# LoganWilliams1/mhm2_kmer_analysis_v2

Measured on AMD Instinct MI355X. Metric: k-mers/sec (kcount stage) at k=21, higher is better.
Workload: dtype u64

## Files before the change

### mhm2_kmer_analysis_v2_amd/csrc/kc_bucketed.hpp

```cpp
#pragma once
#include "kc_kernels.hpp"

namespace kc {

constexpr int WGB = 1024;
constexpr int SUPER_SPAN = 16 * WGB - PRE - POST;
using TileSuper = TileGeo<WGB, SUPER_SPAN>;
static_assert(TileSuper::GPT == 1 && TileSuper::NGROUP == WGB, "one group per thread");
constexpr int PMAX = 1024;
constexpr int GMAX = 512;

template <int NL> struct Rnd {
  static constexpr int RPOS = NL == 1 ? 16 : NL == 2 ? 8 : 4;
  static constexpr int RPOS_READS = NL == 1 ? 8 : NL <= 3 ? 4 : 2;
  static constexpr size_t STAGE = ((size_t)WGB * RPOS + 64) * NL * 8;
  static constexpr size_t STAGE_READS = ((size_t)WGB * RPOS_READS + 64) * NL * 8;
};

struct Geom {
  uint32_t G, P1, P2, S;
  uint32_t log2CH1, log2CH2;
  uint32_t L1MAX, L2MAX;
  uint32_t A1;
  uint32_t A2;
// ... 409 lines not shown
    Lh ^= kc_feistel_f(Rh, 0, K);
    Rh ^= kc_feistel_f(Lh, 1, K);
    Lh ^= kc_feistel_f(Rh, 2, K);
    const uint64_t mix = ((uint64_t)Lh << K) | Rh;
    lo[j] = (uint32_t)mix;
    bk[j] = valid ? ((uint32_t)(mix >> (2 * K - gm.la)) | (le << 10) | (re << 13)) : ~0u;
  }
}

template <int K, int RPOS, class TL>
__device__ __forceinline__ uint32_t cut_run_fixed(const TL &L, int lp0, bool active, uint64_t (&rec)[RPOS], uint64_t (&h)[RPOS]) {
  constexpr int NB = RPOS + K + 1;
  static_assert(NB <= 32 && RPOS % 8 == 0 && PRE % 8 == 0, "the window must fit one word and never start word-aligned");
  const uint64_t *W = reinterpret_cast<const uint64_t *>(L.codes);
  const uint32_t *OK = reinterpret_cast<const uint32_t *>(L.ok);
  const int p = lp0 - 1, q = p >> 5, s = p & 31;
  const uint64_t w0 = W[q], w1 = W[q + 1];
  const uint32_t ok0 = OK[q], ok1 = OK[q + 1], g0 = L.gap[q], g1 = L.gap[q + 1];
  const uint64_t Wn = (w0 << (2 * s)) | (w1 >> (64 - 2 * s));
  const uint32_t nok = ~__builtin_amdgcn_alignbit(ok1, ok0, (uint32_t)s);
  const uint32_t gapw = __builtin_amdgcn_alignbit(g1, g0, (uint32_t)s);
  const uint64_t Rn = kc_rc_word(Wn) << (64 - 2 * NB);
  constexpr uint64_t MID = ((1ULL << (2 * K)) - 1ULL) << 2;
  constexpr uint64_t CMP = (K & 1) ? (MID | 3ULL) : MID;
  uint32_t okm = 0;
#pragma unroll
  for (int j = 0; j < RPOS; j++) {
    const uint64_t x = Wn >> (64 - 2 * (j + K + 2)), y = Rn >> (64 - 2 * (RPOS - 1 - j + K + 2));
    const bool swap = (y & CMP) < (x & CMP);
    const uint64_t sel = swap ? y : x;
    const uint32_t na = (nok >> j) & 1u, nb = (nok >> (j + K + 1)) & 1u;
    const uint32_t le = ((uint32_t)(sel >> (2 * K + 2)) & 3u) | ((swap ? nb : na) << 2);
    const uint32_t re = ((uint32_t)sel & 3u) | ((swap ? na : nb) << 2);
    const uint64_t key = (sel >> 2) << (64 - 2 * K);
    const uint64_t kk[1] = {key};
    h[j] = kc_hash<1>(kk);
    rec[j] = key | (uint64_t)((le & 4u) ? 4u : le) | ((uint64_t)((re & 4u) ? 4u : re) << 3);
    const bool valid = active && ((gapw >> (j + 1)) & ((1u << (K + 1)) - 1u)) == 0u;
    okm |= valid ? (1u << j) : 0u;
  }
  return okm;
}

template <int NL, int FMT, bool CP, bool SH>
__global__ __launch_bounds__(WGB) void kc_l1_reads_kernel(ExtractArgs a, Geom gm, BucketBufs bb, uint64_t nsuper, uint32_t rot,
                                                          uint64_t *ctrs, uint64_t *cb) {
  extern __shared__ __align__(16) uint8_t smem[];
  L1LDS &L = *reinterpret_cast<L1LDS *>(smem);
  uint64_t *sorted = reinterpret_cast<uint64_t *>(smem + ((sizeof(L1LDS) + 15) & ~size_t(15)));
  uint16_t *sbucket = CP ? nullptr : reinterpret_cast<uint16_t *>(smem + ((sizeof(L1LDS) + 15) & ~size_t(15)) + Rnd<NL>::STAGE_READS);
  constexpr int RPOS = Rnd<NL>::RPOS_READS;
  const int tid = threadIdx.x;
  const uint32_t g = (blockIdx.x + rot) % gm.G, P1 = gm.P1;
  ChainDest D = l1_dest<NL>(gm, bb, g);
#ifdef KC_STAMPS
  unsigned long long tprev_ = __builtin_amdgcn_s_memtime();
  D.stamps = cb + 8;
  D.tprev = &tprev_;
#endif
  ChainState cst = split_load_state(L.sp, P1, bb.cnt1 + (size_t)g * P1, D.chain, D.LMAX, D.log2CH, bb.used1[g], bb.used1[gm.G + g]);
  __syncthreads();
  uint32_t n_ins = 0;
  int buf = 0;
  TileRaw<TileSuper> raw;
  auto first_of = [&](uint64_t st) -> uint64_t { return (FMT != FMT_SEQBLOCK && st < nsuper) ? a.tile_first[st] : 0; };
  tile_prefetch<FMT, TileSuper>(raw, a, a.pos0 + (int64_t)blockIdx.x * SUPER_SPAN, tid, first_of(blockIdx.x), blockIdx.x < nsuper);
  uint64_t next_first = first_of((uint64_t)blockIdx.x + gridDim.x);
  constexpr int RUNS = SUPER_SPAN / RPOS;
  static_assert(SUPER_SPAN % RPOS == 0, "runs must tile the span");
  constexpr int NROUND = (RUNS + WGB - 1) / WGB;
  for (int64_t it = -1;; it++) {
    const uint64_t st = (uint64_t)blockIdx.x + (uint64_t)(it < 0 ? 0 : it) * gridDim.x;
    const bool work = it >= 0;
    if (work && st >= nsuper) break;
#pragma unroll 1
    for (int round = 0; round < NROUND; round++) {
      uint64_t rec[RPOS][NL];
      uint32_t br[RPOS];
      uint32_t total = 0;
      if (work) {
      const int run_id = round * WGB + tid;
      const bool active = run_id < RUNS;
      const int lp0 = PRE + (active ? run_id : 0) * RPOS;
      KmerRun<NL> run;
      run_begin<NL>(run, L.tile, lp0, a.k);
#pragma unroll
      for (int j = 0; j < RPOS; j++) {
        uint64_t h = 0;
        uint32_t owner = 0;
        bool valid = run_kmer<NL, !CP>(run, j, lp0, a.k, rec[j], h, SH ? a.rank_n : 1u, SH ? a.reference_owner : 0u, SH ? &owner : nullptr) && active;
        if (SH) {
          if (CP && !a.reference_owner) {
            uint64_t key[NL];
#pragma unroll
            for (int w = 0; w < NL; w++) key[w] = rec[j][w];
            key[NL - 1] &= ~KC_EXT_MASK;
            owner = kc_owner_of_hash(kc_hash<NL>(key), a.rank_n);
          }
          valid = valid && owner == a.rank_me;
        }
        if (CP) rec[j][0] = cp_mix_rec(rec[j][0], gm);
        br[j] = valid ? (CP ? cp_b1(rec[j][0], gm) : hash_b1(h, gm)) : ~0u;
        if (j + 1 < RPOS) run_advance<NL>(run, j, lp0, a.k);
      }
#pragma unroll
      for (int j = 0; j < RPOS; j++) {
        const bool valid = br[j] != ~0u;
        const uint32_t rank = hist_rank(L.sp, buf, br[j] & (PMAX - 1), valid);
        br[j] = valid ? (br[j] | (rank << 10)) : ~0u;
        n_ins += valid ? 1u : 0u;
      }
      KC_SPLIT_STAMP(0)
      lds_barrier();
      total = split_stage<NL, RPOS>(
          L.sp, sorted, sbucket, buf, P1,
          [&](int j, uint64_t (&o)[NL]) {
#pragma unroll
            for (int w = 0; w < NL; w++) o[w] = rec[j][w];
          },
          br, D, cst);
      }
      if (round == NROUND - 1) {
        const uint64_t nst = work ? st + gridDim.x : st;
        tile_encode<FMT, TileSuper>(L.tile, raw, a, a.pos0 + (int64_t)nst * SUPER_SPAN, ctrs, tid, nst < nsuper);
        tile_prefetch<FMT, TileSuper>(raw, a, a.pos0 + (int64_t)(nst + gridDim.x) * SUPER_SPAN, tid, next_first, nst + gridDim.x < nsuper);
        next_first = first_of(nst + 2 * (uint64_t)gridDim.x);
        KC_SPLIT_STAMP(5)
      }
      if (work) {
        split_copy_out<NL>(
            L.sp, sorted, sbucket, total, D, [&](const uint64_t (&r)[NL]) { return cp_b1(r[0], gm); },
            [&](uint32_t, const uint64_t (&r)[NL]) { l1_overflow<NL, CP>(gm, bb, cb, r); },
            [&](size_t i, const uint64_t (&r)[NL]) { store_words<NL>(D.arena, i, r); });
        buf ^= 1;
      }
    }
  }
  if ((uint32_t)tid < P1) bb.cnt1[(size_t)g * P1 + tid] = cst.cur;
  if (tid == 0) {
    bb.used1[g] = min(L.sp.arena_used, gm.A1);
    bb.used1[gm.G + g] = min(L.sp.arena_top, gm.A1);
  }
  for (int o = 32; o > 0; o >>= 1) n_ins += __shfl_down(n_ins, o);
  if (lane_id() == 0 && n_ins) atomicAdd((unsigned long long *)&ctrs[CTR_INSERTED], (unsigned long long)n_ins);
}

constexpr int R16 = 16;
constexpr uint32_t ST16_MAIN = (uint32_t)WGB * R16 + PMAX;
constexpr uint32_t ST16_SLOTS = ST16_MAIN + 64;
static_assert(SUPER_SPAN % R16 == 0 && SUPER_SPAN / R16 <= WGB, "one run of sixteen positions per thread covers the super-tile");
static_assert(ST16_MAIN < 65536, "staging positions fit 16 bits");
constexpr size_t l1x16_lds_bytes() { return ((sizeof(L1LDS) + 15) & ~size_t(15)) + (size_t)ST16_SLOTS * 6; }

template <class MidFn>
__device__ __forceinline__ uint32_t split_stage_pairs(SplitLDS &L, uint32_t *slo, uint16_t *sbk, int buf, uint32_t P, const uint32_t (&lo)[R16],
                                                      const uint32_t (&br)[R16], const ChainDest &D, ChainState &st, MidFn mid) {
  const int tid = fresh_tid();
  KC_SPLIT_STAMP(1)
  const uint32_t v = ((uint32_t)tid < P) ? L.hist[buf][tid] : 0u;
  const uint32_t excl = block_excl_scan((v + 1u) & ~1u, L.scan);
  const uint32_t CHm = (1u << D.log2CH) - 1u;
  if ((uint32_t)tid < P) {
    const uint32_t base = st.cur;
    uint32_t fit = v;
    const uint64_t room = ((uint64_t)D.LMAX << D.log2CH) - base;
    if ((uint64_t)fit > room) fit = (uint32_t)room;
    const uint32_t have = (base + CHm) >> D.log2CH;
    uint32_t k = ((base + fit + CHm) >> D.log2CH) - have, a = 0;
    if (k) {
      const bool own = (uint32_t)tid >= D.own_lo && (uint32_t)tid < D.own_hi;
      if (own) {
        a = atomicAdd(&L.arena_used, k);
        const uint32_t left = D.arena_cap - min(D.arena_cap, L.arena_top);
        if (a + k > left) {
          k = a < left ? left - a : 0;
          const uint64_t cap = ((uint64_t)(have + k) << D.log2CH) - base;
          if ((uint64_t)fit > cap) fit = (uint32_t)cap;
        }
      } else {
        const uint32_t t = atomicAdd(&L.arena_top, k);
        const uint32_t left = D.arena_cap - min(D.arena_cap, L.arena_used);
        if (t + k > left) {
          k = 0;
          const uint64_t cap = ((uint64_t)have << D.log2CH) - base;
          if ((uint64_t)fit > cap) fit = (uint32_t)cap;
        } else {
          a = D.arena_cap - t - k;
        }
      }
      uint32_t *ch = D.chain + (size_t)tid * D.LMAX + have;
      for (uint32_t i = 0; i < k; i++) ch[i] = D.arena_base + a + i;
    }
    uint4 d;
    d.x = ((st.last - D.arena_base - (base >> D.log2CH)) << D.log2CH) + base - excl;
    d.y = ((a - have) << D.log2CH) + base - excl;
    d.z = excl | (v << 16);
    d.w = fit | (((base & CHm) ? min(fit, (CHm + 1u) - (base & CHm)) : 0u) << 16);
    L.dst[tid] = d;
    if (k) st.last = D.arena_base + a + k - 1;
    st.cur = base + fit;
    L.hist[buf][tid] = excl;
    L.hist[buf ^ 1][tid] = 0;
  }
  lds_barrier();
  KC_SPLIT_STAMP(2)
  const uint32_t total = L.scan.total;
#pragma unroll
  for (int j0 = 0; j0 < R16; j0 += 8) {
    uint32_t pos[8];
#pragma unroll
    for (int j = 0; j < 8; j++) pos[j] = L.hist[buf][br[j0 + j] & (PMAX - 1)];
#pragma unroll
    for (int j = 0; j < 8; j++) {
      const uint32_t bj = br[j0 + j];
      const uint32_t p = bj != ~0u ? pos[j] + (bj >> 16) : ST16_MAIN + lane_id();
      slo[p] = lo[j0 + j];
      sbk[p] = (uint16_t)bj;
    }
  }
  mid();
  lds_barrier();
  KC_SPLIT_STAMP(3)
  return total;
}

struct __attribute__((packed, aligned(2))) Rec6Pair {
  uint32_t w0, w1, w2;
};
struct __attribute__((packed, aligned(2))) Rec6 {
  uint32_t lo;
  uint16_t bk;
};
static_assert(sizeof(Rec6Pair) == 12 && sizeof(Rec6) == 6, "six bytes a record");

template <class OvfFn>
__device__ __forceinline__ void split_copy_out_pairs(SplitLDS &L, const uint32_t *slo, const uint16_t *sbk, uint32_t total, const ChainDest &D,
                                                     const Geom &gm, OvfFn overflow) {
  const int tid = fresh_tid();
  constexpr int U = 2;
  uint8_t *const arena0 = reinterpret_cast<uint8_t *>(D.arena) + ((size_t)D.arena_base << D.log2CH) * 6;
  const uint32_t shb = 64u - gm.la, shl = 64u - gm.k2;
  for (uint32_t i0 = 2u * (uint32_t)tid; i0 < total; i0 += 2u * U * WGB) {
    uint64_t lo2[U];
    uint32_t bk2[U];
    uint4 d[U];
#pragma unroll
    for (int u = 0; u < U; u++) {
      const uint32_t i = i0 + 2u * (uint32_t)u * WGB;
      const uint32_t ii = i < total ? i : i0;
      lo2[u] = *reinterpret_cast<const uint64_t *>(slo + ii);
      bk2[u] = *reinterpret_cast<const uint32_t *>(sbk + ii);
    }
#pragma unroll
    for (int u = 0; u < U; u++) d[u] = L.dst[bk2[u] & (PMAX - 1)];
    bool odd = false;
#pragma unroll
    for (int u = 0; u < U; u++) {
      const uint32_t i = i0 + 2u * (uint32_t)u * WGB;
      const uint32_t j = i - (d[u].z & 0xFFFFu), v = d[u].z >> 16, fit = d[u].w & 0xFFFFu, wold = d[u].w >> 16;
      const bool live = i < total;
      const bool f0 = live && j < fit, real1 = live && j + 1u < v, f1 = real1 && j + 1u < fit;
      const uint32_t at0 = (j < wold ? d[u].x : d[u].y) + i, at1 = (j + 1u < wold ? d[u].x : d[u].y) + i + 1u;
      const bool pair = f0 && f1 && at1 == at0 + 1u;
      if (pair) {
        const uint32_t l1 = (uint32_t)(lo2[u] >> 32);
        Rec6Pair r;
        r.w0 = (uint32_t)lo2[u];
        r.w1 = (bk2[u] & 0xFFFFu) | (l1 << 16);
        r.w2 = (l1 >> 16) | (bk2[u] & 0xFFFF0000u);
        *reinterpret_cast<Rec6Pair *>(arena0 + (size_t)at0 * 6) = r;
      } else if (f0) {
        Rec6 r;
        r.lo = (uint32_t)lo2[u];
        r.bk = (uint16_t)bk2[u];
        *reinterpret_cast<Rec6 *>(arena0 + (size_t)at0 * 6) = r;
      }
      odd |= (real1 && !pair) || (live && !f0);
    }
    if (__any(odd)) {
#pragma unroll
      for (int u = 0; u < U; u++) {
        const uint32_t i = i0 + 2u * (uint32_t)u * WGB;
        if (i >= total) continue;
        const uint32_t j = i - (d[u].z & 0xFFFFu), v = d[u].z >> 16, fit = d[u].w & 0xFFFFu, wold = d[u].w >> 16;
        const uint32_t at0 = (j < wold ? d[u].x : d[u].y) + i, at1 = (j + 1u < wold ? d[u].x : d[u].y) + i + 1u;
        const uint32_t l0 = (uint32_t)lo2[u], l1 = (uint32_t)(lo2[u] >> 32);
        const uint64_t bh = (uint64_t)(bk2[u] & (PMAX - 1)) << shb;
        const uint64_t ra = bh | ((uint64_t)l0 << shl) | (uint64_t)((bk2[u] >> 10) & 63u);
        const uint64_t rb = bh | ((uint64_t)l1 << shl) | (uint64_t)(bk2[u] >> 26);
        const bool f0 = j < fit, real1 = j + 1u < v, f1 = real1 && j + 1u < fit;
        if (!f0) overflow(ra);
        if (real1 && !(f0 && f1 && at1 == at0 + 1u)) {
          if (f1) {
            Rec6 r;
            r.lo = l1;
            r.bk = (uint16_t)(bk2[u] >> 16);
            *reinterpret_cast<Rec6 *>(arena0 + (size_t)at1 * 6) = r;
          } else {
            overflow(rb);
          }
        }
      }
    }
  }
  KC_SPLIT_STAMP(4)
}

template <int FMT, bool SH, int KK>
__global__ __launch_bounds__(WGB) void kc_l1_reads16_kernel(ExtractArgs a, Geom gm, BucketBufs bb, uint64_t nsuper, uint32_t rot, uint64_t *ctrs,
                                                            uint64_t *cb) {
  extern __shared__ __align__(16) uint8_t smem[];
  L1LDS &L = *reinterpret_cast<L1LDS *>(smem);
  uint32_t *slo = reinterpret_cast<uint32_t *>(smem + ((sizeof(L1LDS) + 15) & ~size_t(15)));
  uint16_t *sbk = reinterpret_cast<uint16_t *>(slo + ST16_SLOTS);
  const int tid = threadIdx.x;
  const uint32_t g = (blockIdx.x + rot) % gm.G, P1 = gm.P1;
  ChainDest D = l1_dest6(gm, bb, g);
#ifdef KC_STAMPS
  unsigned long long tprev_ = __builtin_amdgcn_s_memtime();
  D.stamps = cb + 8;
  D.tprev = &tprev_;
#endif
  ChainState cst = split_load_state(L.sp, P1, bb.cnt1 + (size_t)g * P1, D.chain, D.LMAX, D.log2CH, bb.used1[g], bb.used1[gm.G + g]);
  __syncthreads();
  uint32_t n_ins = 0;
  int buf = 0;
  TileRaw<TileSuper> raw;
  auto first_of = [&](uint64_t st) -> uint64_t { return (FMT != FMT_SEQBLOCK && st < nsuper) ? a.tile_first[st] : 0; };
  tile_prefetch<FMT, TileSuper>(raw, a, a.pos0 + (int64_t)blockIdx.x * SUPER_SPAN, tid, first_of(blockIdx.x), blockIdx.x < nsuper);
  uint64_t next_first = first_of((uint64_t)blockIdx.x + gridDim.x);
  constexpr int RUNS = SUPER_SPAN / R16;
  {
    const int ft = fresh_tid();
    tile_encode<FMT, TileSuper>(L.tile, raw, a, a.pos0 + (int64_t)blockIdx.x * SUPER_SPAN, ctrs, ft, blockIdx.x < nsuper);
    tile_prefetch<FMT, TileSuper>(raw, a, a.pos0 + (int64_t)((uint64_t)blockIdx.x + gridDim.x) * SUPER_SPAN, ft, next_first,
                                  (uint64_t)blockIdx.x + gridDim.x < nsuper);
    next_first = first_of((uint64_t)blockIdx.x + 2 * (uint64_t)gridDim.x);
  }
  for (uint64_t st = blockIdx.x; st < nsuper; st += gridDim.x) {
    uint32_t lo[R16], br[R16];
    const bool active = tid < RUNS;
    const int lp0 = PRE + (active ? tid : 0) * R16;
    {
      uint32_t l8[8], b8[8];
      cp_run_fixed<KK, 8, SH>(L.tile, lp0, active, gm, a, l8, b8);
#pragma unroll
      for (int j = 0; j < 8; j++) {
        lo[j] = l8[j];
        br[j] = b8[j];
      }
      cp_run_fixed<KK, 8, SH>(L.tile, lp0 + 8, active, gm, a, l8, b8);
#pragma unroll
      for (int j = 0; j < 8; j++) {
        lo[8 + j] = l8[j];
        br[8 + j] = b8[j];
      }
    }
#pragma unroll
    for (int j = 0; j < R16; j++) {
      const bool valid = br[j] != ~0u;
      const uint32_t rank = hist_rank(L.sp, buf, br[j] & (PMAX - 1), valid);
      br[j] = valid ? (br[j] | (rank << 16)) : ~0u;
      n_ins += valid ? 1u : 0u;
    }
    KC_SPLIT_STAMP(0)
    lds_barrier();
    const int ft = fresh_tid();
    const uint64_t nst = st + gridDim.x;
    tile_encode_clear<TileSuper>(L.tile, raw, ft);
    const uint32_t total = split_stage_pairs(L.sp, slo, sbk, buf, P1, lo, br, D, cst, [&]() {
      tile_encode_fill<FMT, TileSuper>(L.tile, raw, a, a.pos0 + (int64_t)nst * SUPER_SPAN, ctrs, ft, nst < nsuper);
      tile_prefetch<FMT, TileSuper>(raw, a, a.pos0 + (int64_t)(nst + gridDim.x) * SUPER_SPAN, ft, next_first, nst + gridDim.x < nsuper);
      next_first = first_of(nst + 2 * (uint64_t)gridDim.x);
    });
    split_copy_out_pairs(L.sp, slo, sbk, total, D, gm, [&](uint64_t r) {
      const uint64_t rr[1] = {r};
      l1_overflow<1, true>(gm, bb, cb, rr);
    });
    buf ^= 1;
  }
  if ((uint32_t)tid < P1) bb.cnt1[(size_t)g * P1 + tid] = cst.cur;
  if (tid == 0) {
    bb.used1[g] = min(L.sp.arena_used, gm.A1);
    bb.used1[gm.G + g] = min(L.sp.arena_top, gm.A1);
  }
  for (int o = 32; o > 0; o >>= 1) n_ins += __shfl_down(n_ins, o);
  if (lane_id() == 0 && n_ins) atomicAdd((unsigned long long *)&ctrs[CTR_INSERTED], (unsigned long long)n_ins);
}

template <int NL, int R>
__device__ __forceinline__ void split_round_flat(SplitLDS &L, int buf, uint32_t P, const uint64_t (&rec)[R][NL], const uint32_t (&br)[R],
                                                 uint64_t *records, uint64_t seg_cap, uint64_t *cursors, uint64_t *overflow_flag) {
  const int tid = threadIdx.x;
  if ((uint32_t)tid < P) {
    const uint32_t v = L.hist[buf][tid];
    uint64_t base = 0;
    if (v) base = atomicAdd((unsigned long long *)&cursors[tid], (unsigned long long)v);
    const uint64_t room = base < seg_cap ? seg_cap - base : 0;
    uint4 d;
    d.x = (uint32_t)base;
    d.y = (uint32_t)(base >> 32);
    d.z = (uint64_t)v <= room ? v : (uint32_t)room;
    d.w = 0;
    L.dst[tid] = d;
    L.hist[buf ^ 1][tid] = 0;
  }
  lds_barrier();
#pragma unroll
  for (int j = 0; j < R; j++) {
    if (br[j] != ~0u) {
      const uint32_t b = br[j] & (PMAX - 1), rank = br[j] >> 10;
      const uint4 d = L.dst[b];
      if (rank < d.z) {
        uint64_t *o = records + ((uint64_t)b * seg_cap + (((uint64_t)d.y << 32) | d.x) + rank) * NL;
#pragma unroll
        for (int w = 0; w < NL; w++) o[w] = rec[j][w];
      } else {
        *overflow_flag = 1;
      }
    }
  }
}

template <int NL, int FMT>
__global__ __launch_bounds__(WGB) void kc_bin_reads_kernel(ExtractArgs a, uint64_t nsuper, uint64_t *ctrs) {
  extern __shared__ __align__(16) uint8_t smem[];
  L1LDS &L = *reinterpret_cast<L1LDS *>(smem);
  constexpr int RPOS = Rnd<NL>::RPOS_READS;
  const int tid = threadIdx.x;
  const uint32_t P = a.rank_n;
  if ((uint32_t)tid < PMAX) {
    L.sp.hist[0][tid] = 0;
    L.sp.hist[1][tid] = 0;
  }
  __syncthreads();
  int buf = 0;
  TileRaw<TileSuper> raw;
  auto first_of = [&](uint64_t st) -> uint64_t { return (FMT != FMT_SEQBLOCK && st < nsuper) ? a.tile_first[st] : 0; };
  tile_prefetch<FMT, TileSuper>(raw, a, a.pos0 + (int64_t)blockIdx.x * SUPER_SPAN, tid, first_of(blockIdx.x), blockIdx.x < nsuper);
  uint64_t next_first = first_of((uint64_t)blockIdx.x + gridDim.x);
  constexpr int RUNS = SUPER_SPAN / RPOS;
  static_assert(SUPER_SPAN % RPOS == 0, "runs must tile the span");
  for (uint64_t st = blockIdx.x; st < nsuper; st += gridDim.x) {
    const int64_t T0 = a.pos0 + (int64_t)st * SUPER_SPAN;
    tile_encode<FMT, TileSuper>(L.tile, raw, a, T0, ctrs, tid, true);
    {
      const uint64_t nst = st + gridDim.x;
      tile_prefetch<FMT, TileSuper>(raw, a, a.pos0 + (int64_t)nst * SUPER_SPAN, tid, next_first, nst < nsuper);
      next_first = first_of(nst + gridDim.x);
    }
#pragma unroll 1
    for (int round = 0; round < (RUNS + WGB - 1) / WGB; round++) {
      uint64_t rec[RPOS][NL];
// ... 1492 lines not shown
```

### mhm2_kmer_analysis_v2_amd/csrc/kc_kernels.hpp

```cpp
#pragma once
#include "kc_common.hpp"

namespace kc {

constexpr int TPB = 256;
constexpr int PPT = 16;
constexpr int TILE = TPB * PPT;
constexpr int PRE = 32;
constexpr int POST = 192;
template <int THREADS_, int SPAN_>
struct TileGeo {
  static constexpr int THREADS = THREADS_;
  static constexpr int SPAN = SPAN_;
  static constexpr int LSPAN = PRE + SPAN_ + POST;
  static constexpr int NGROUP = LSPAN / 16;
  static constexpr int NWORD = LSPAN / 32;
  static constexpr int GPT = (NGROUP + THREADS_ - 1) / THREADS_;
  static_assert(LSPAN % 32 == 0, "staged span must be whole words");
};
using TileSmall = TileGeo<TPB, TILE>;

constexpr uint64_t KEY_EMPTY = ~0ULL;
constexpr uint64_t KEY_BUSY = ~0ULL - 1;
constexpr uint64_t KEY_NEVER = ~0ULL - 2;

enum { MODE_INSERT = 0, MODE_BIN = 1 };
enum { FMT_READS = 0, FMT_SEQBLOCK = 1, FMT_PACKED = 2, FMT_READS_UQ = 3 };
constexpr bool fmt_is_reads(int fmt) { return fmt == FMT_READS || fmt == FMT_READS_UQ; }

enum {
  CTR_ENTRIES = 0,
  CTR_INSERTED,
  CTR_BAD_BASE,
  CTR_OUT,
  CTR_PURGED,
  CTR_SUM_COUNTS,
  CTR_RAW_KMERS,
  CTR_EXPECT,
  CTR_OVERFLOW,
  CTR_BIN0,
  CTR_COUNT = CTR_BIN0 + 64
};

struct Table {
  uint64_t *keys;
  uint32_t *vals;
  uint64_t mask;
};

struct ExtractArgs {
  const uint8_t *bases;
  const uint8_t *quals;
  const uint64_t *offsets;
  const uint64_t *tile_first;
  uint64_t nreads;
  uint64_t total;
  uint32_t align;
  int64_t pos0;
  int k;
  int qual_cut;
  uint32_t rank_me, rank_n;
  uint32_t reference_owner;
  uint64_t *records;
  uint64_t seg_capacity;
};

__device__ __forceinline__ uint32_t lane_id() { return __lane_id(); }

__device__ __forceinline__ void sat_inc(uint32_t *p) {
  uint32_t old = atomicAdd(p, 1u);
  if (old >= 0x80000000u) atomicSub(p, 1u);
}

template <int NL>
__device__ __forceinline__ uint64_t table_slot(const Table &t, const uint64_t (&key)[NL], bool &is_new) {
  uint64_t slot = kc_hash<NL>(key) & t.mask;
  is_new = false;
  if constexpr (NL == 1) {
    for (;;) {
      uint64_t cur = t.keys[slot];
      if (cur == key[0]) break;
      if (cur == KEY_EMPTY) {
        uint64_t old = atomicCAS((unsigned long long *)&t.keys[slot], (unsigned long long)KEY_EMPTY,
                                 (unsigned long long)key[0]);
        if (old == KEY_EMPTY) { is_new = true; break; }
        if (old == key[0]) break;
      }
      slot = (slot + 1) & t.mask;
    }
  } else {
    bool done = false;
    do {
      unsigned long long *ks = (unsigned long long *)(t.keys + slot * NL);
      unsigned long long old = KEY_BUSY;
      if (!done) old = atomicCAS(&ks[NL - 1], (unsigned long long)KEY_EMPTY, (unsigned long long)KEY_BUSY);
      const bool won = !done && old == KEY_EMPTY;
      if (won) {
#pragma unroll
        for (int j = 0; j < NL - 1; j++)
          __hip_atomic_store(&ks[j], (unsigned long long)key[j], __ATOMIC_RELAXED, __HIP_MEMORY_SCOPE_AGENT);
        asm volatile("s_waitcnt vmcnt(0)" ::: "memory");
        atomicExch(&ks[NL - 1], (unsigned long long)key[NL - 1]);
        is_new = true;
      }
      bool same = !done && old == key[NL - 1];
      if (same) {
#pragma unroll
        for (int j = 0; j < NL - 1; j++) same &= (atomicOr(&ks[j], 0ULL) == key[j]);
      }
      const bool busy = !done && old == KEY_BUSY;
      if (!done && !won && !same && !busy) slot = (slot + 1) & t.mask;
      done = done || won || same;
    } while (__any(!done));
  }
  return slot;
}

template <int NL>
__device__ __forceinline__ void table_insert(const Table &t, const uint64_t (&rec)[NL], uint64_t *ctrs) {
  uint64_t key[NL];
#pragma unroll
  for (int j = 0; j < NL; j++) key[j] = rec[j];
  const uint32_t le = (uint32_t)(rec[NL - 1] & 7u), re = (uint32_t)((rec[NL - 1] >> 3) & 7u);
  key[NL - 1] &= ~KC_EXT_MASK;
  bool is_new;
  const uint64_t slot = table_slot<NL>(t, key, is_new);
  uint32_t *v = t.vals + slot * 9;
  sat_inc(v);
  if (le < 4u) sat_inc(v + 1 + le);
  if (re < 4u) sat_inc(v + 5 + re);
  if (is_new) atomicAdd((unsigned long long *)&ctrs[CTR_ENTRIES], 1ULL);
}

__device__ __forceinline__ void sat_add(uint32_t *p, uint32_t x) {
  if (!x) return;
  const uint32_t old = atomicAdd(p, x);
  if (old >= 0x80000000u) atomicSub(p, x);
}
template <int NL>
__global__ __launch_bounds__(TPB) void kc_merge_entries_kernel(const uint64_t *keys, const uint16_t *counts, const uint16_t *exts, uint64_t n,
                                                               Table t, uint64_t *ctrs) {
  for (uint64_t i = (uint64_t)blockIdx.x * TPB + threadIdx.x; i < n; i += (uint64_t)gridDim.x * TPB) {
    uint64_t key[NL];
#pragma unroll
    for (int j = 0; j < NL; j++) key[j] = keys[i * NL + j];
    bool is_new;
    const uint64_t slot = table_slot<NL>(t, key, is_new);
    uint32_t *v = t.vals + slot * 9;
    sat_add(v, counts[i]);
#pragma unroll
    for (int x = 0; x < 8; x++) sat_add(v + 1 + x, exts[i * 8 + x]);
    if (is_new) atomicAdd((unsigned long long *)&ctrs[CTR_ENTRIES], 1ULL);
  }
}

template <class G>
struct alignas(16) TileLDS {
  uint32_t codes[G::NGROUP];
  uint16_t ok[G::NGROUP];
  uint32_t gap[G::NWORD + 1];
  uint64_t far_off;
};

__device__ __forceinline__ uint32_t pack4(uint32_t v) {
  uint32_t b = (v >> 1) & 0x03030303u;
  uint32_t c = b ^ ((b >> 1) & 0x01010101u);
  return (c * 0x40100401u) >> 24;
}

__device__ __forceinline__ uint32_t pack4_cache(uint32_t v) {
  uint32_t c = (v & 0x03030303u) | ((v >> 1) & 0x02020202u);
  return (c * 0x40100401u) >> 24;
}

constexpr uint32_t BM_ACGT = (1u << 1) | (1u << 3) | (1u << 7) | (1u << 20);
constexpr uint32_t BM_ACGTN = BM_ACGT | (1u << 14);
__device__ __forceinline__ bool in_bitmap(uint32_t c, uint32_t bm) { return ((c & 0xC0u) == 0x40u) && ((bm >> (c & 31u)) & 1u); }

__device__ __forceinline__ uint32_t nz7(uint32_t x) { return ((x & 0x7F7F7F7Fu) + 0x7F7F7F7Fu) | x; }
template <int FMT>
__device__ __forceinline__ void encode_group_swar(const uint32_t (&bw)[4], const uint32_t (&qw)[4], uint32_t qual_cut, uint32_t &okm,
                                                  uint32_t &sepm, bool &bad) {
  uint32_t badacc = 0, ok_lo = 0, ok_hi = 0, sp_lo = 0, sp_hi = 0;
#pragma unroll
  for (int j = 0; j < 4; j++) {
    const uint32_t w = bw[j];
    const uint32_t weight = (j & 1) ? 0x80402010u : 0x08040201u;
    uint32_t ok, sp = 0;
    if (FMT == FMT_PACKED) {
      const uint32_t x = w & ((w << 1) | (w << 2));
      badacc |= x << 5;
      ok = x & ~(w << 5);
    } else {
      const uint32_t u = w & 0xDFDFDFDFu;
      const uint32_t not_acgt = nz7(u ^ 0x41414141u) & nz7(u ^ 0x43434343u) & nz7(u ^ 0x47474747u) & nz7(u ^ 0x54545454u);
      const uint32_t not_n = nz7(u ^ 0x4E4E4E4Eu);
      uint32_t hq;
      if (fmt_is_reads(FMT)) {
        const uint32_t q = qw[j];
        hq = (((q & 0x7F7F7F7Fu) | 0x80808080u) - qual_cut * 0x01010101u) | q;
        badacc |= not_acgt & not_n;
      } else {
        hq = ~(w << 2);
        const uint32_t not_sep = nz7(w ^ 0x5F5F5F5Fu);
        sp = ~not_sep;
        badacc |= not_acgt & not_n & not_sep;
      }
      ok = hq & ~not_acgt;
    }
    if (j < 2) {
      ok_lo = __builtin_amdgcn_udot4(ok & 0x80808080u, weight, ok_lo, false);
      if (FMT == FMT_SEQBLOCK) sp_lo = __builtin_amdgcn_udot4(sp & 0x80808080u, weight, sp_lo, false);
    } else {
      ok_hi = __builtin_amdgcn_udot4(ok & 0x80808080u, weight, ok_hi, false);
      if (FMT == FMT_SEQBLOCK) sp_hi = __builtin_amdgcn_udot4(sp & 0x80808080u, weight, sp_hi, false);
    }
  }
  okm = (ok_lo >> 7) | ((ok_hi >> 7) << 8);
  if (FMT == FMT_SEQBLOCK) sepm = (sp_lo >> 7) | ((sp_hi >> 7) << 8);
  if (badacc & 0x80808080u) bad = true;
}

__device__ __forceinline__ void tile_barrier() { asm volatile("s_waitcnt lgkmcnt(0)\n\ts_barrier" ::: "memory"); }

template <class G>
struct TileRaw {
  uint32_t bw[G::GPT][4];
  uint32_t qw[G::GPT][4];
  uint64_t first_read;
  uint64_t off;
};

template <int FMT, class G>
__device__ __forceinline__ void tile_prefetch(TileRaw<G> &R, const ExtractArgs &a, int64_t T0, int tid, uint64_t tile_first_read, bool active) {
  const int64_t lo = a.align, hi = (int64_t)a.align + (int64_t)a.total;
#pragma unroll
  for (int gi = 0; gi < G::GPT; gi++) {
#pragma unroll
    for (int w = 0; w < 4; w++) {
      R.bw[gi][w] = 0;
      R.qw[gi][w] = 0;
    }
    const int g = tid + gi * G::THREADS;
    const int64_t X0 = T0 - PRE + 16 * g;
    if (active && g < G::NGROUP && (X0 + 16 > lo) && (X0 < hi)) {
      const uint4 v = *reinterpret_cast<const uint4 *>(a.bases + X0);
      R.bw[gi][0] = v.x; R.bw[gi][1] = v.y; R.bw[gi][2] = v.z; R.bw[gi][3] = v.w;
      if (fmt_is_reads(FMT)) {
        if (FMT == FMT_READS) {
          const uint4 q = *reinterpret_cast<const uint4 *>(a.quals + X0);
          R.qw[gi][0] = q.x; R.qw[gi][1] = q.y; R.qw[gi][2] = q.z; R.qw[gi][3] = q.w;
        } else {
          for (int i = 0; i < 16; i++) {
            const int64_t x = X0 + i;
            if (x >= lo && x < hi) R.qw[gi][i >> 2] |= (uint32_t)a.quals[x] << (8 * (i & 3));
          }
        }
      }
    }
  }
  R.first_read = tile_first_read;
  R.off = ~0ULL;
  if (FMT != FMT_SEQBLOCK && active && tile_first_read + tid <= a.nreads) R.off = a.offsets[tile_first_read + tid];
}

template <class G>
__device__ __forceinline__ void tile_encode_clear(TileLDS<G> &L, const TileRaw<G> &R, int tid) {
  for (int i = tid; i < G::NWORD + 1; i += G::THREADS) L.gap[i] = 0;
  if (tid == G::THREADS - 1) L.far_off = R.off;
}
template <int FMT, class G>
__device__ __forceinline__ void tile_encode_fill(TileLDS<G> &L, const TileRaw<G> &R, const ExtractArgs &a, int64_t T0, uint64_t *ctrs, int tid,
                                                 bool active);

template <int FMT, class G>
__device__ __forceinline__ void tile_encode(TileLDS<G> &L, const TileRaw<G> &R, const ExtractArgs &a, int64_t T0, uint64_t *ctrs, int tid,
                                            bool active) {
  tile_encode_clear<G>(L, R, tid);
  tile_barrier();
  tile_encode_fill<FMT, G>(L, R, a, T0, ctrs, tid, active);
  tile_barrier();
}

template <int FMT, class G>
__device__ __forceinline__ void tile_encode_fill(TileLDS<G> &L, const TileRaw<G> &R, const ExtractArgs &a, int64_t T0, uint64_t *ctrs, int tid,
                                                 bool active) {
#ifdef KC_STAMPS
  unsigned long long ts_ = __builtin_amdgcn_s_memtime();
#define KC_ENC_STAMP(k)                                                              \
  if (threadIdx.x == 0) {                                                            \
    const unsigned long long tn_ = __builtin_amdgcn_s_memtime();                     \
    atomicAdd((unsigned long long *)&ctrs[CTR_BIN0 + 40 + k], tn_ - ts_);            \
    ts_ = tn_;                                                                       \
  }
#else
#define KC_ENC_STAMP(k)
#endif
  KC_ENC_STAMP(0)
  if (!active) return;
  const int64_t lo = a.align, hi = (int64_t)a.align + (int64_t)a.total;
  bool bad = false;
#pragma unroll
  for (int gi = 0; gi < G::GPT; gi++) {
    const int g = tid + gi * G::THREADS;
    if (g >= G::NGROUP) break;
    const int64_t X0 = T0 - PRE + 16 * g;
    const uint32_t(&bw)[4] = R.bw[gi];
    const uint32_t(&qw)[4] = R.qw[gi];
    const bool any = (X0 + 16 > lo) && (X0 < hi);
    const bool full = (X0 >= lo) && (X0 + 16 <= hi);
    uint32_t code = FMT == FMT_PACKED ? (pack4_cache(bw[0]) << 24) | (pack4_cache(bw[1]) << 16) | (pack4_cache(bw[2]) << 8) | pack4_cache(bw[3])
                                      : (pack4(bw[0]) << 24) | (pack4(bw[1]) << 16) | (pack4(bw[2]) << 8) | pack4(bw[3]);
    uint32_t okm = 0, sepm = 0;
    if (full && (!fmt_is_reads(FMT) || a.qual_cut <= 128)) {
      encode_group_swar<FMT>(bw, qw, (uint32_t)a.qual_cut, okm, sepm, bad);
    } else {
#pragma unroll
      for (int j = 0; j < 4; j++) {
        uint32_t wb = bw[j], wq = qw[j];
#pragma unroll 1
        for (int i = 4 * j; i < 4 * j + 4; i++, wb >>= 8, wq >>= 8) {
          const uint32_t c = wb & 0xFFu;
          const bool real = full || (any && (X0 + i >= lo) && (X0 + i < hi));
          bool hq;
          if (FMT == FMT_PACKED) {
            hq = (c >> 3) >= KC_QUAL_CUTOFF;
            if (real && (c & 7u) > 4u) bad = true;
            if (real && hq && (c & 7u) < 4u) okm |= 1u << i;
            continue;
          }
          if (fmt_is_reads(FMT)) {
            const int q = (int)(wq & 0xFFu);
            hq = q >= a.qual_cut;
            if (real && !in_bitmap(c, BM_ACGTN)) bad = true;
          } else {
            hq = (c & 0x20u) == 0;
            const bool sep = (c == '_');
            if (real && sep) sepm |= 1u << i;
            if (real && !sep && !in_bitmap(c, BM_ACGTN)) bad = true;
          }
          if (real && hq && in_bitmap(c, BM_ACGT)) okm |= 1u << i;
        }
      }
    }
    L.codes[g ^ 1] = code;
    L.ok[g] = (uint16_t)okm;
    if (!full) {
      uint32_t nonreal = 0xFFFFu;
      if (any) {
        const int i0 = (int)(lo > X0 ? lo - X0 : 0), i1 = (int)(hi - X0 < 16 ? hi - X0 : 16);
        nonreal = ~(((1u << i1) - 1u) & ~((1u << i0) - 1u)) & 0xFFFFu;
      }
      atomicOr(&L.gap[g >> 1], nonreal << (16 * (g & 1)));
    }
    if (FMT == FMT_SEQBLOCK && sepm) {
      uint64_t bits = ((uint64_t)sepm | ((uint64_t)sepm << 1)) << (16 * (g & 1));
      atomicOr(&L.gap[g >> 1], (uint32_t)bits);
      if (bits >> 32) atomicOr(&L.gap[(g >> 1) + 1], (uint32_t)(bits >> 32));
    }
  }
  KC_ENC_STAMP(1)
  if (FMT != FMT_SEQBLOCK) {
    const int64_t first = T0, last = T0 + G::SPAN + a.k;
    const uint64_t far = L.far_off;
    const bool more = far != ~0ULL && (int64_t)far + lo <= last;
    uint64_t off = R.off;
    for (uint64_t r = R.first_read + tid; r <= a.nreads; r += G::THREADS) {
      if (r != R.first_read + tid) off = a.offsets[r];
      const int64_t s = (int64_t)off + lo;
      if (s > last) break;
      if (s >= first) {
        const int lp = (int)(s - (T0 - PRE));
        atomicOr(&L.gap[lp >> 5], 1u << (lp & 31));
      }
      if (!more) break;
    }
  } else {
    if (tid == 0) {
      int64_t s0 = lo - (T0 - PRE), s1 = hi - (T0 - PRE);
      if (s0 >= 0 && s0 < G::LSPAN) atomicOr(&L.gap[s0 >> 5], 1u << (s0 & 31));
      if (s1 >= 0 && s1 < G::LSPAN) atomicOr(&L.gap[s1 >> 5], 1u << (s1 & 31));
    }
  }
  if (bad) ctrs[CTR_BAD_BASE] = 1;
  KC_ENC_STAMP(2)
}

template <int FMT, class G>
__device__ __forceinline__ void stage_tile(TileLDS<G> &L, const ExtractArgs &a, int64_t T0, uint64_t *ctrs, int tid, uint64_t tile_first_read,
                                           bool active) {
  TileRaw<G> R;
  tile_prefetch<FMT, G>(R, a, T0, tid, tile_first_read, active);
  tile_encode<FMT, G>(L, R, a, T0, ctrs, tid, active);
}

template <int NL, class TL>
__device__ __forceinline__ bool tile_kmer(const TL &L, int lp, int k, uint64_t (&rec)[NL], uint64_t &h, uint32_t rank_n = 1,
                                          uint32_t reference_owner = 0, uint32_t *owner = nullptr) {
  {
    int rem = k + 1, w = lp >> 5, s = lp & 31;
    uint32_t badbits = L.gap[w] >> s;
    int got = 32 - s;
    if (got >= rem) {
      if (rem < 32) badbits &= (1u << rem) - 1u;
    } else {
      rem -= got;
      w++;
      while (rem >= 32) { badbits |= L.gap[w++]; rem -= 32; }
      if (rem) badbits |= L.gap[w] & ((1u << rem) - 1u);
    }
    if (badbits) return false;
  }
  const uint64_t *W = reinterpret_cast<const uint64_t *>(L.codes);
  const int q = lp >> 5, sh = 2 * (lp & 31);
  uint64_t f[NL], r[NL];
#pragma unroll
  for (int j = 0; j < NL; j++) {
    uint64_t hi = W[q + j], lo = W[q + j + 1];
    f[j] = (sh ? ((hi << sh) | (lo >> (64 - sh))) : hi) & kc_word_mask(k, j);
  }
  kc_revcomp<NL>(f, k, r);
  const int pl = lp - 1, pr = lp + k;
  uint32_t lc = (uint32_t)(W[pl >> 5] >> (62 - 2 * (pl & 31))) & 3u;
  uint32_t rc = (uint32_t)(W[pr >> 5] >> (62 - 2 * (pr & 31))) & 3u;
  uint32_t le = ((L.ok[pl >> 4] >> (pl & 15)) & 1u) ? lc : KC_EXT_NONE;
  uint32_t re = ((L.ok[pr >> 4] >> (pr & 15)) & 1u) ? rc : KC_EXT_NONE;
  if (owner) *owner = 0;
  if (owner && rank_n > 1 && reference_owner) *owner = kc_reference_owner<NL>(f, r, k, rank_n);
  if (kc_less<NL>(r, f)) {
#pragma unroll
    for (int j = 0; j < NL; j++) f[j] = r[j];
    uint32_t nl = (re == KC_EXT_NONE) ? KC_EXT_NONE : 3u - re;
    uint32_t nr = (le == KC_EXT_NONE) ? KC_EXT_NONE : 3u - le;
    le = nl;
    re = nr;
  }
  h = kc_hash<NL>(f);
  if (owner && rank_n > 1 && !reference_owner) *owner = kc_owner_of_hash(h, rank_n);
#pragma unroll
  for (int j = 0; j < NL; j++) rec[j] = f[j];
  rec[NL - 1] |= (uint64_t)(le | (re << 3));
  return true;
}

template <int NL>
struct KmerRun {
  uint64_t f[NL], r[NL];
  uint64_t nextb;
  uint32_t okl, okr;
  uint32_t gin;
  uint32_t lc;
  int lastgap;
};

template <int NL, class TL>
__device__ __forceinline__ void run_begin(KmerRun<NL> &s, const TL &L, int lp0, int k) {
  const uint64_t *W = reinterpret_cast<const uint64_t *>(L.codes);
  {
    const int q = lp0 >> 5, sh = 2 * (lp0 & 31);
#pragma unroll
    for (int j = 0; j < NL; j++) {
      const uint64_t hi = W[q + j], lo = W[q + j + 1];
      s.f[j] = (sh ? ((hi << sh) | (lo >> (64 - sh))) : hi) & kc_word_mask(k, j);
    }
  }
  kc_revcomp<NL>(s.f, k, s.r);
  const int pl = lp0 - 1, pr = lp0 + k;
  {
    const int q = pr >> 5, sh = 2 * (pr & 31);
    const uint64_t hi = W[q], lo = W[q + 1];
    s.nextb = sh ? ((hi << sh) | (lo >> (64 - sh))) : hi;
  }
  s.lc = (uint32_t)(W[pl >> 5] >> (62 - 2 * (pl & 31))) & 3u;
  s.okl = ((uint32_t)L.ok[pl >> 4] | ((uint32_t)L.ok[(pl >> 4) + 1] << 16)) >> (pl & 15);
  s.okr = ((uint32_t)L.ok[pr >> 4] | ((uint32_t)L.ok[(pr >> 4) + 1] << 16)) >> (pr & 15);
  {
    const int a = pr + 1, w = a >> 5, sh = a & 31;
    const uint32_t g0 = L.gap[w], g1 = L.gap[w + 1];
    s.gin = sh ? ((g0 >> sh) | (g1 << (32 - sh))) : g0;
  }
  int last = -1;
  const int w0 = lp0 >> 5, w1 = pr >> 5;
  for (int w = w0; w <= w1; w++) {
    uint32_t bits = L.gap[w];
    if (w == w0) bits &= ~0u << (lp0 & 31);
    if (w == w1 && (pr & 31) < 31) bits &= (2u << (pr & 31)) - 1u;
    if (bits) last = 32 * w + 31 - __clz(bits);
  }
  s.lastgap = last;
}

template <int NL, bool HASH = true>
__device__ __forceinline__ bool run_kmer(const KmerRun<NL> &s, int j, int lp0, int k, uint64_t (&rec)[NL], uint64_t &h, uint32_t rank_n = 1,
                                         uint32_t reference_owner = 0, uint32_t *owner = nullptr) {
  const uint32_t c = (uint32_t)(s.nextb >> 62);
  uint32_t le = ((s.okl >> j) & 1u) ? s.lc : KC_EXT_NONE;
// ... 333 lines not shown
```

Baseline: 100.1 billion.

## Add simple-bucket fast path in copy-out and cheaper SWAR base encoding

During staging, each bucket destination is flagged as simple when all of its records fit and none straddle a partially filled chunk. When every lane in a wave sees only simple buckets, copy-out takes a fast path that writes paired or single six-byte records from a single base offset. This skips the per-record fit, wrap and pairing checks. Separately, the encode step moves into a new header. The 2-bit packing now uses udot4, the ACGT check uses a perm-table lookup, and the N and separator classification is deferred to a wave-uniform slow path that runs only when some character is not ACGT.

```diff
diff --git a/mhm2_kmer_analysis_v2_amd/csrc/kc_bucketed.hpp b/mhm2_kmer_analysis_v2_amd/csrc/kc_bucketed.hpp
--- a/mhm2_kmer_analysis_v2_amd/csrc/kc_bucketed.hpp
+++ b/mhm2_kmer_analysis_v2_amd/csrc/kc_bucketed.hpp
@@ -585,6 +585,7 @@
 static_assert(ST16_MAIN < 65536, "staging positions fit 16 bits");
 constexpr size_t l1x16_lds_bytes() { return ((sizeof(L1LDS) + 15) & ~size_t(15)) + (size_t)ST16_SLOTS * 6; }
 
+constexpr uint32_t DST_SIMPLE = 0x80000000u;
 template <class MidFn>
 __device__ __forceinline__ uint32_t split_stage_pairs(SplitLDS &L, uint32_t *slo, uint16_t *sbk, int buf, uint32_t P, const uint32_t (&lo)[R16],
                                                       const uint32_t (&br)[R16], const ChainDest &D, ChainState &st, MidFn mid) {
@@ -624,11 +625,16 @@
       uint32_t *ch = D.chain + (size_t)tid * D.LMAX + have;
       for (uint32_t i = 0; i < k; i++) ch[i] = D.arena_base + a + i;
     }
+    const uint32_t wold = (base & CHm) ? min(fit, (CHm + 1u) - (base & CHm)) : 0u;
+    const bool simple = fit == v && (wold == 0u || wold >= v);
+    uint32_t flag = simple ? 1u : 0u;
+    asm("" : "+v"(flag));
     uint4 d;
     d.x = ((st.last - D.arena_base - (base >> D.log2CH)) << D.log2CH) + base - excl;
     d.y = ((a - have) << D.log2CH) + base - excl;
-    d.z = excl | (v << 16);
-    d.w = fit | (((base & CHm) ? min(fit, (CHm + 1u) - (base & CHm)) : 0u) << 16);
+    if (simple && !wold) d.x = d.y;
+    d.z = excl | (v << 16) | (flag << 31);
+    d.w = fit | (wold << 16);
     L.dst[tid] = d;
     if (k) st.last = D.arena_base + a + k - 1;
     st.cur = base + fit;
@@ -665,6 +671,20 @@
   uint16_t bk;
 };
 static_assert(sizeof(Rec6Pair) == 12 && sizeof(Rec6) == 6, "six bytes a record");
+__device__ __forceinline__ void store_rec6_pair(uint8_t *arena0, uint32_t at, uint64_t lo2, uint32_t bk2) {
+  const uint32_t l1 = (uint32_t)(lo2 >> 32);
+  Rec6Pair r;
+  r.w0 = (uint32_t)lo2;
+  r.w1 = (bk2 & 0xFFFFu) | (l1 << 16);
+  r.w2 = (l1 >> 16) | (bk2 & 0xFFFF0000u);
+  *reinterpret_cast<Rec6Pair *>(arena0 + (size_t)at * 6) = r;
+}
+__device__ __forceinline__ void store_rec6(uint8_t *arena0, uint32_t at, uint32_t lo, uint32_t bk) {
+  Rec6 r;
+  r.lo = lo;
+  r.bk = (uint16_t)bk;
+  *reinterpret_cast<Rec6 *>(arena0 + (size_t)at * 6) = r;
+}
 
 template <class OvfFn>
 __device__ __forceinline__ void split_copy_out_pairs(SplitLDS &L, const uint32_t *slo, const uint16_t *sbk, uint32_t total, const ChainDest &D,
@@ -686,28 +706,31 @@
     }
 #pragma unroll
     for (int u = 0; u < U; u++) d[u] = L.dst[bk2[u] & (PMAX - 1)];
+    bool simple = true;
+#pragma unroll
+    for (int u = 0; u < U; u++) simple = simple && (i0 + 2u * (uint32_t)u * WGB >= total || (d[u].z & DST_SIMPLE));
+    if (__all(simple)) {
+#pragma unroll
+      for (int u = 0; u < U; u++) {
+        const uint32_t i = i0 + 2u * (uint32_t)u * WGB;
+        if (i >= total) continue;
+        const uint32_t j = i - (d[u].z & 0xFFFFu), v = (d[u].z >> 16) & 0x7FFFu, at0 = d[u].x + i;
+        if (j + 1u < v) store_rec6_pair(arena0, at0, lo2[u], bk2[u]);
+        else store_rec6(arena0, at0, (uint32_t)lo2[u], bk2[u]);
+      }
+      continue;
+    }
     bool odd = false;
 #pragma unroll
     for (int u = 0; u < U; u++) {
       const uint32_t i = i0 + 2u * (uint32_t)u * WGB;
-      const uint32_t j = i - (d[u].z & 0xFFFFu), v = d[u].z >> 16, fit = d[u].w & 0xFFFFu, wold = d[u].w >> 16;
+      const uint32_t j = i - (d[u].z & 0xFFFFu), v = (d[u].z >> 16) & 0x7FFFu, fit = d[u].w & 0xFFFFu, wold = d[u].w >> 16;
       const bool live = i < total;
       const bool f0 = live && j < fit, real1 = live && j + 1u < v, f1 = real1 && j + 1u < fit;
       const uint32_t at0 = (j < wold ? d[u].x : d[u].y) + i, at1 = (j + 1u < wold ? d[u].x : d[u].y) + i + 1u;
       const bool pair = f0 && f1 && at1 == at0 + 1u;
-      if (pair) {
-        const uint32_t l1 = (uint32_t)(lo2[u] >> 32);
-        Rec6Pair r;
-        r.w0 = (uint32_t)lo2[u];
-        r.w1 = (bk2[u] & 0xFFFFu) | (l1 << 16);
-        r.w2 = (l1 >> 16) | (bk2[u] & 0xFFFF0000u);
-        *reinterpret_cast<Rec6Pair *>(arena0 + (size_t)at0 * 6) = r;
-      } else if (f0) {
-        Rec6 r;
-        r.lo = (uint32_t)lo2[u];
-        r.bk = (uint16_t)bk2[u];
-        *reinterpret_cast<Rec6 *>(arena0 + (size_t)at0 * 6) = r;
-      }
+      if (pair) store_rec6_pair(arena0, at0, lo2[u], bk2[u]);
+      else if (f0) store_rec6(arena0, at0, (uint32_t)lo2[u], bk2[u]);
       odd |= (real1 && !pair) || (live && !f0);
     }
     if (__any(odd)) {
@@ -715,7 +738,7 @@
       for (int u = 0; u < U; u++) {
         const uint32_t i = i0 + 2u * (uint32_t)u * WGB;
         if (i >= total) continue;
-        const uint32_t j = i - (d[u].z & 0xFFFFu), v = d[u].z >> 16, fit = d[u].w & 0xFFFFu, wold = d[u].w >> 16;
+        const uint32_t j = i - (d[u].z & 0xFFFFu), v = (d[u].z >> 16) & 0x7FFFu, fit = d[u].w & 0xFFFFu, wold = d[u].w >> 16;
         const uint32_t at0 = (j < wold ? d[u].x : d[u].y) + i, at1 = (j + 1u < wold ? d[u].x : d[u].y) + i + 1u;
         const uint32_t l0 = (uint32_t)lo2[u], l1 = (uint32_t)(lo2[u] >> 32);
         const uint64_t bh = (uint64_t)(bk2[u] & (PMAX - 1)) << shb;
@@ -724,14 +747,8 @@
         const bool f0 = j < fit, real1 = j + 1u < v, f1 = real1 && j + 1u < fit;
         if (!f0) overflow(ra);
         if (real1 && !(f0 && f1 && at1 == at0 + 1u)) {
-          if (f1) {
-            Rec6 r;
-            r.lo = l1;
-            r.bk = (uint16_t)(bk2[u] >> 16);
-            *reinterpret_cast<Rec6 *>(arena0 + (size_t)at1 * 6) = r;
-          } else {
-            overflow(rb);
-          }
+          if (f1) store_rec6(arena0, at1, l1, bk2[u] >> 16);
+          else overflow(rb);
         }
       }
     }
diff --git a/mhm2_kmer_analysis_v2_amd/csrc/kc_encode.hpp b/mhm2_kmer_analysis_v2_amd/csrc/kc_encode.hpp
--- /dev/null
+++ b/mhm2_kmer_analysis_v2_amd/csrc/kc_encode.hpp
@@ -0,0 +1,150 @@
+#pragma once
+#include "kc_common.hpp"
+
+namespace kc {
+
+enum { FMT_READS = 0, FMT_SEQBLOCK = 1, FMT_PACKED = 2, FMT_READS_UQ = 3 };
+constexpr bool fmt_is_reads(int fmt) { return fmt == FMT_READS || fmt == FMT_READS_UQ; }
+
+KC_HD uint32_t kc_udot4(uint32_t a, uint32_t b, uint32_t c) {
+#if defined(__HIP_DEVICE_COMPILE__)
+  return __builtin_amdgcn_udot4(a, b, c, false);
+#else
+  for (int i = 0; i < 4; i++) c += ((a >> (8 * i)) & 0xFFu) * ((b >> (8 * i)) & 0xFFu);
+  return c;
+#endif
+}
+template <uint32_t tab>
+KC_HD uint32_t kc_perm4(uint32_t sel) {
+#if defined(__HIP_DEVICE_COMPILE__)
+  uint32_t t;
+  asm("s_mov_b32 %0, %1" : "=s"(t) : "i"(tab));
+  return __builtin_amdgcn_perm(0u, t, sel);
+#else
+  uint32_t r = 0;
+  for (int i = 0; i < 4; i++) r |= ((tab >> (8 * ((sel >> (8 * i)) & 3u))) & 0xFFu) << (8 * i);
+  return r;
+#endif
+}
+KC_HD bool kc_wave_any(bool x) {
+#if defined(__HIP_DEVICE_COMPILE__)
+  return __any(x) != 0;
+#else
+  return x;
+#endif
+}
+
+constexpr uint32_t GATHER2 = 0x01041040u;
+KC_HD uint32_t gray4(uint32_t v) { return (v >> 1) & 0x03030303u; }
+KC_HD uint32_t pack16(const uint32_t (&bw)[4]) {
+  const uint32_t g0 = kc_udot4(gray4(bw[0]), GATHER2, 0u), g1 = kc_udot4(gray4(bw[1]), GATHER2, 0u);
+  const uint32_t g2 = kc_udot4(gray4(bw[2]), GATHER2, 0u), g3 = kc_udot4(gray4(bw[3]), GATHER2, 0u);
+  const uint32_t g = (g0 << 24) | (g1 << 16) | (g2 << 8) | g3;
+  return g ^ ((g >> 1) & 0x55555555u);
+}
+KC_HD uint32_t pack4_cache(uint32_t v) {
+  return kc_udot4((v & 0x03030303u) | ((v >> 1) & 0x02020202u), GATHER2, 0u);
+}
+KC_HD uint32_t pack16_cache(const uint32_t (&bw)[4]) {
+  return (pack4_cache(bw[0]) << 24) | (pack4_cache(bw[1]) << 16) | (pack4_cache(bw[2]) << 8) | pack4_cache(bw[3]);
+}
+template <int FMT>
+KC_HD uint32_t encode_group_codes(const uint32_t (&bw)[4]) {
+  return FMT == FMT_PACKED ? pack16_cache(bw) : pack16(bw);
+}
+
+constexpr uint32_t BM_ACGT = (1u << 1) | (1u << 3) | (1u << 7) | (1u << 20);
+constexpr uint32_t BM_ACGTN = BM_ACGT | (1u << 14);
+KC_HD bool in_bitmap(uint32_t c, uint32_t bm) { return ((c & 0xC0u) == 0x40u) && ((bm >> (c & 31u)) & 1u); }
+
+template <int FMT>
+KC_HD void encode_group_edge(const uint32_t (&bw)[4], const uint32_t (&qw)[4], int qual_cut, int64_t X0, int64_t lo, int64_t hi,
+                             uint32_t &okm, uint32_t &sepm, bool &bad) {
+  const bool any = (X0 + 16 > lo) && (X0 < hi);
+  const bool full = (X0 >= lo) && (X0 + 16 <= hi);
+#pragma unroll
+  for (int j = 0; j < 4; j++) {
+    uint32_t wb = bw[j], wq = qw[j];
+#pragma unroll 1
+    for (int i = 4 * j; i < 4 * j + 4; i++, wb >>= 8, wq >>= 8) {
+      const uint32_t c = wb & 0xFFu;
+      const bool real = full || (any && (X0 + i >= lo) && (X0 + i < hi));
+      bool hq;
+      if (FMT == FMT_PACKED) {
+        hq = (c >> 3) >= KC_QUAL_CUTOFF;
+        if (real && (c & 7u) > 4u) bad = true;
+        if (real && hq && (c & 7u) < 4u) okm |= 1u << i;
+        continue;
+      }
+      if (fmt_is_reads(FMT)) {
+        const int q = (int)(wq & 0xFFu);
+        hq = q >= qual_cut;
+        if (real && !in_bitmap(c, BM_ACGTN)) bad = true;
+      } else {
+        hq = (c & 0x20u) == 0;
+        const bool sep = (c == '_');
+        if (real && sep) sepm |= 1u << i;
+        if (real && !sep && !in_bitmap(c, BM_ACGTN)) bad = true;
+      }
+      if (real && hq && in_bitmap(c, BM_ACGT)) okm |= 1u << i;
+    }
+  }
+}
+
+KC_HD uint32_t nz7(uint32_t x) { return ((x & 0x7F7F7F7Fu) + 0x7F7F7F7Fu) | x; }
+KC_HD uint32_t not_acgt7(uint32_t w) { return nz7((w & 0xDFDFDFDFu) ^ kc_perm4<0x47544341u>(gray4(w))); }
+
+template <int FMT>
+KC_HD void encode_group_swar(const uint32_t (&bw)[4], const uint32_t (&qw)[4], uint32_t qual_cut, uint32_t &okm, uint32_t &sepm,
+                             bool &bad) {
+  uint32_t badacc = 0, ok_lo = 0, ok_hi = 0;
+  const uint32_t cut4 = qual_cut * 0x01010101u;
+#pragma unroll
+  for (int j = 0; j < 4; j++) {
+    const uint32_t w = bw[j];
+    const uint32_t weight = (j & 1) ? 0x80402010u : 0x08040201u;
+    uint32_t ok;
+    if (FMT == FMT_PACKED) {
+      const uint32_t x = w & ((w << 1) | (w << 2));
+      badacc |= x << 5;
+      ok = x & ~(w << 5);
+    } else {
+      const uint32_t na = not_acgt7(w);
+      uint32_t hq;
+      if (fmt_is_reads(FMT)) {
+        const uint32_t q = qw[j];
+        hq = (((q & 0x7F7F7F7Fu) | 0x80808080u) - cut4) | q;
+      } else {
+        hq = ~(w << 2);
+      }
+      badacc |= na;
+      ok = hq & ~na;
+    }
+    if (j < 2) ok_lo = kc_udot4(ok & 0x80808080u, weight, ok_lo);
+    else ok_hi = kc_udot4(ok & 0x80808080u, weight, ok_hi);
+  }
+  okm = (ok_lo >> 7) | ((ok_hi >> 7) << 8);
+  if (FMT == FMT_PACKED) {
+    if (badacc & 0x80808080u) bad = true;
+  } else if (kc_wave_any((badacc & 0x80808080u) != 0)) {
+    uint32_t sp_lo = 0, sp_hi = 0;
+    badacc = 0;
+#pragma unroll
+    for (int j = 0; j < 4; j++) {
+      const uint32_t w = bw[j];
+      const uint32_t weight = (j & 1) ? 0x80402010u : 0x08040201u;
+      uint32_t other = not_acgt7(w) & nz7((w & 0xDFDFDFDFu) ^ 0x4E4E4E4Eu);
+      if (FMT == FMT_SEQBLOCK) {
+        const uint32_t not_sep = nz7(w ^ 0x5F5F5F5Fu);
+        other &= not_sep;
+        if (j < 2) sp_lo = kc_udot4(~not_sep & 0x80808080u, weight, sp_lo);
+        else sp_hi = kc_udot4(~not_sep & 0x80808080u, weight, sp_hi);
+      }
+      badacc |= other;
+    }
+    if (FMT == FMT_SEQBLOCK) sepm = (sp_lo >> 7) | ((sp_hi >> 7) << 8);
+    if (badacc & 0x80808080u) bad = true;
+  }
+}
+
+}
diff --git a/mhm2_kmer_analysis_v2_amd/csrc/kc_kernels.hpp b/mhm2_kmer_analysis_v2_amd/csrc/kc_kernels.hpp
--- a/mhm2_kmer_analysis_v2_amd/csrc/kc_kernels.hpp
+++ b/mhm2_kmer_analysis_v2_amd/csrc/kc_kernels.hpp
@@ -1,5 +1,6 @@
 #pragma once
 #include "kc_common.hpp"
+#include "kc_encode.hpp"
 
 namespace kc {
 
@@ -25,8 +26,6 @@
 constexpr uint64_t KEY_NEVER = ~0ULL - 2;
 
 enum { MODE_INSERT = 0, MODE_BIN = 1 };
-enum { FMT_READS = 0, FMT_SEQBLOCK = 1, FMT_PACKED = 2, FMT_READS_UQ = 3 };
-constexpr bool fmt_is_reads(int fmt) { return fmt == FMT_READS || fmt == FMT_READS_UQ; }
 
 enum {
   CTR_ENTRIES = 0,
@@ -162,64 +161,6 @@
   uint64_t far_off;
 };
 
-__device__ __forceinline__ uint32_t pack4(uint32_t v) {
-  uint32_t b = (v >> 1) & 0x03030303u;
-  uint32_t c = b ^ ((b >> 1) & 0x01010101u);
-  return (c * 0x40100401u) >> 24;
-}
-
-__device__ __forceinline__ uint32_t pack4_cache(uint32_t v) {
-  uint32_t c = (v & 0x03030303u) | ((v >> 1) & 0x02020202u);
-  return (c * 0x40100401u) >> 24;
-}
-
-constexpr uint32_t BM_ACGT = (1u << 1) | (1u << 3) | (1u << 7) | (1u << 20);
-constexpr uint32_t BM_ACGTN = BM_ACGT | (1u << 14);
-__device__ __forceinline__ bool in_bitmap(uint32_t c, uint32_t bm) { return ((c & 0xC0u) == 0x40u) && ((bm >> (c & 31u)) & 1u); }
-
-__device__ __forceinline__ uint32_t nz7(uint32_t x) { return ((x & 0x7F7F7F7Fu) + 0x7F7F7F7Fu) | x; }
-template <int FMT>
-__device__ __forceinline__ void encode_group_swar(const uint32_t (&bw)[4], const uint32_t (&qw)[4], uint32_t qual_cut, uint32_t &okm,
-                                                  uint32_t &sepm, bool &bad) {
-  uint32_t badacc = 0, ok_lo = 0, ok_hi = 0, sp_lo = 0, sp_hi = 0;
-#pragma unroll
-  for (int j = 0; j < 4; j++) {
-    const uint32_t w = bw[j];
-    const uint32_t weight = (j & 1) ? 0x80402010u : 0x08040201u;
-    uint32_t ok, sp = 0;
-    if (FMT == FMT_PACKED) {
-      const uint32_t x = w & ((w << 1) | (w << 2));
-      badacc |= x << 5;
-      ok = x & ~(w << 5);
-    } else {
-      const uint32_t u = w & 0xDFDFDFDFu;
-      const uint32_t not_acgt = nz7(u ^ 0x41414141u) & nz7(u ^ 0x43434343u) & nz7(u ^ 0x47474747u) & nz7(u ^ 0x54545454u);
-      const uint32_t not_n = nz7(u ^ 0x4E4E4E4Eu);
-      uint32_t hq;
-      if (fmt_is_reads(FMT)) {
-        const uint32_t q = qw[j];
-        hq = (((q & 0x7F7F7F7Fu) | 0x80808080u) - qual_cut * 0x01010101u) | q;
-        badacc |= not_acgt & not_n;
-      } else {
-        hq = ~(w << 2);
-        const uint32_t not_sep = nz7(w ^ 0x5F5F5F5Fu);
-        sp = ~not_sep;
-        badacc |= not_acgt & not_n & not_sep;
-      }
-      ok = hq & ~not_acgt;
-    }
-    if (j < 2) {
-      ok_lo = __builtin_amdgcn_udot4(ok & 0x80808080u, weight, ok_lo, false);
-      if (FMT == FMT_SEQBLOCK) sp_lo = __builtin_amdgcn_udot4(sp & 0x80808080u, weight, sp_lo, false);
-    } else {
-      ok_hi = __builtin_amdgcn_udot4(ok & 0x80808080u, weight, ok_hi, false);
-      if (FMT == FMT_SEQBLOCK) sp_hi = __builtin_amdgcn_udot4(sp & 0x80808080u, weight, sp_hi, false);
-    }
-  }
-  okm = (ok_lo >> 7) | ((ok_hi >> 7) << 8);
-  if (FMT == FMT_SEQBLOCK) sepm = (sp_lo >> 7) | ((sp_hi >> 7) << 8);
-  if (badacc & 0x80808080u) bad = true;
-}
 
 __device__ __forceinline__ void tile_barrier() { asm volatile("s_waitcnt lgkmcnt(0)\n\ts_barrier" ::: "memory"); }
 
@@ -309,39 +250,12 @@
     const uint32_t(&qw)[4] = R.qw[gi];
     const bool any = (X0 + 16 > lo) && (X0 < hi);
     const bool full = (X0 >= lo) && (X0 + 16 <= hi);
-    uint32_t code = FMT == FMT_PACKED ? (pack4_cache(bw[0]) << 24) | (pack4_cache(bw[1]) << 16) | (pack4_cache(bw[2]) << 8) | pack4_cache(bw[3])
-                                      : (pack4(bw[0]) << 24) | (pack4(bw[1]) << 16) | (pack4(bw[2]) << 8) | pack4(bw[3]);
+    const uint32_t code = encode_group_codes<FMT>(bw);
     uint32_t okm = 0, sepm = 0;
     if (full && (!fmt_is_reads(FMT) || a.qual_cut <= 128)) {
       encode_group_swar<FMT>(bw, qw, (uint32_t)a.qual_cut, okm, sepm, bad);
     } else {
-#pragma unroll
-      for (int j = 0; j < 4; j++) {
-        uint32_t wb = bw[j], wq = qw[j];
-#pragma unroll 1
-        for (int i = 4 * j; i < 4 * j + 4; i++, wb >>= 8, wq >>= 8) {
-          const uint32_t c = wb & 0xFFu;
-          const bool real = full || (any && (X0 + i >= lo) && (X0 + i < hi));
-          bool hq;
-          if (FMT == FMT_PACKED) {
-            hq = (c >> 3) >= KC_QUAL_CUTOFF;
-            if (real && (c & 7u) > 4u) bad = true;
-            if (real && hq && (c & 7u) < 4u) okm |= 1u << i;
-            continue;
-          }
-          if (fmt_is_reads(FMT)) {
-            const int q = (int)(wq & 0xFFu);
-            hq = q >= a.qual_cut;
-            if (real && !in_bitmap(c, BM_ACGTN)) bad = true;
-          } else {
-            hq = (c & 0x20u) == 0;
-            const bool sep = (c == '_');
-            if (real && sep) sepm |= 1u << i;
-            if (real && !sep && !in_bitmap(c, BM_ACGTN)) bad = true;
-          }
-          if (real && hq && in_bitmap(c, BM_ACGT)) okm |= 1u << i;
-        }
-      }
+      encode_group_edge<FMT>(bw, qw, a.qual_cut, X0, lo, hi, okm, sepm, bad);
     }
     L.codes[g ^ 1] = code;
     L.ok[g] = (uint16_t)okm;
```

Result: faster. 103.8 billion (median of 6 runs) (+3.7%).
